# adjerbetian/OpenCL_PathTracer

Hardware: AMD Instinct MI355X
Metric: Msamples/s (paths x bounces) at 1920x1080 (higher is better)
Workload: dtype f32; 1 GPU; BASELINE configs[2]: synthetic random-triangle scene (numpy MT19937 seed 12345): 1000000 triangles (665533 BVH nodes, depth 22), 1920x1080, ray depth 10, JITTERED, 1 light(s); spp_total=256, parallelism=single GPU

## Files before the change

### opencl_pathtracer_amd/csrc/kernel_wavefront.hip

```cpp
#include <hip/hip_runtime.h>

#include "ptmi_device.hpp"
#include "ptmi_shading.hpp"
#include "ptmi_literal_path.hpp"

#include <atomic>
#include <cstdlib>
#include <cstring>

namespace PTMI_DEV_NS {

constexpr int kWfBlock = 256;
constexpr int kWfBlockNarrow = 64;
constexpr int kWfStack = PTMI_BVH_MAX_DEPTH;
#ifndef PTMI_WF_MIN_WAVES
#define PTMI_WF_MIN_WAVES 5
#endif
#ifndef PTMI_WF_MIN_WAVES_GENERAL
#define PTMI_WF_MIN_WAVES_GENERAL 5
#endif
#ifndef PTMI_WF_QUEUES
#define PTMI_WF_QUEUES 8
#endif
constexpr int kQueues = PTMI_WF_QUEUES;
#ifndef PTMI_WF_QUEUE_STRIDE
#define PTMI_WF_QUEUE_STRIDE 64
#endif
constexpr int kQueueStride = PTMI_WF_QUEUE_STRIDE;
static_assert(kQueueStride >= 2, "job_counter[1] is the given-up flag: queue counters must not be adjacent words");
constexpr int kHitRecordWords = 4;
#ifndef PTMI_WF_LEAF_LANES
#define PTMI_WF_LEAF_LANES 19
#endif
#ifndef PTMI_WF_LEAF_RATIO
#define PTMI_WF_LEAF_RATIO 2
#endif
constexpr int kLeafLanes = PTMI_WF_LEAF_LANES, kLeafRatio = PTMI_WF_LEAF_RATIO;
constexpr int kPassWordsPerLane = 4;

struct DWarm {
    const DNode* nodes;
    const DTri* tris;
    const DBigLeaf* big_leaves;
    const uint32_t* tri_ids;
    const DShade* shade;
    const DMat* mats;
    const ptmi_light* lights;
    const ptmi_texture* textures;
    const ptmi_uchar4* texels;
    uint32_t root_ref;
    uint32_t width, height;
    uint32_t max_depth, n_lights, sampler, tris_precomputed;
    uint32_t histograms;
    uint32_t boxes_ordered;
    uint32_t wide_records;
    uint32_t russian_roulette;
    uint32_t source_seed;
    uint32_t wait_debt;
    uint32_t split_paths;
};

constexpr uint32_t kStatDepthBins = 64;
constexpr uint32_t kPoisonMarker = 0x7FC0DEADu;
constexpr uint32_t kGivenUp = 0x80000000u, kGiveUpListFirst = (uint32_t)(kQueues * kQueueStride), kGiveUpListCap = 8u * 1024u - kGiveUpListFirst;
static_assert(kQueues * kQueueStride <= 1024, "the give-up list lies behind the queue counters inside the set's 8 x 1024 dwords");
constexpr uint32_t kSplitWords = C_TRI + 1;
static_assert(PTMI_COUNTER_SPLITS * (int)kSplitWords <= 64, "flushed by one wave");
__device__ __forceinline__ uint32_t counter_split_of(uint32_t slot, uint32_t split_paths)
{
    const uint32_t t1 = split_paths ? split_paths : 0xFFFFFFFFu, t2 = split_paths ? 2u * split_paths : 0xFFFFFFFFu,
                   t3 = split_paths ? 3u * split_paths : 0xFFFFFFFFu;
    return (slot >= t1 ? 1u : 0u) + (slot >= t2 ? 1u : 0u) + (slot >= t3 ? 1u : 0u);
}

__device__ __forceinline__ uint32_t pack_path_statistics(uint32_t depth, uint32_t bbx, uint32_t tri)
{
    static_assert(PTMI_MAX_INTERSECTION_NUMBER <= 8191, "13-bit fields");
    const uint32_t b = bbx < PTMI_MAX_INTERSECTION_NUMBER ? bbx : 8191u, t = tri < PTMI_MAX_INTERSECTION_NUMBER ? tri : 8191u;
    return depth | (b << 6) | (t << 19);
}

__device__ __forceinline__ void decode_leaf(const DWarm& sc, uint32_t ref, uint32_t& tri_i, uint32_t& tri_end)
{
    uint32_t count = (ref >> REF_COUNT_SHIFT) & 7u;
    uint32_t start = ref & REF_INDEX_MASK_LEAF;
    if (count == REF_COUNT_BIG) {
        const DBigLeaf bl = sc.big_leaves[start];
        start = bl.start;
        count = bl.count;
    }
    tri_i = start;
    tri_end = start + count;
}

__device__ __forceinline__ void add_retraced_totals(unsigned long long* totals, uint32_t depth, uint32_t n_seg, uint32_t n_shadow,
                                                    const PathCounters& pc)
{
    atomicAdd(&totals[C_PATHS], 1ull);
    atomicAdd(&totals[C_SEGMENTS], (unsigned long long)n_seg - 1ull);
    atomicAdd(&totals[C_HITS], (unsigned long long)depth);
    atomicAdd(&totals[C_SHADOW], (unsigned long long)n_shadow);
    atomicAdd(&totals[C_BBX], (unsigned long long)pc.bbx);
    atomicAdd(&totals[C_TRI], (unsigned long long)pc.tri);
}

__device__ __forceinline__ void give_path_up(V4& radiance, V4& transfer, uint32_t& reflection, uint32_t& p_bbx, uint32_t& p_tri)
{
    const float m = __uint_as_float(kPoisonMarker);
    radiance = v4(m, m, m, m);
    transfer = v4(1, 1, 1, 1);
    reflection = 0; p_bbx = 0; p_tri = 0;
}

template <bool STATS, bool PRE, bool SS, bool PLAIN = false, bool NANSAFE = false, int BLOCK = 256>
__global__ void __launch_bounds__(BLOCK, PLAIN ? PTMI_WF_MIN_WAVES : PTMI_WF_MIN_WAVES_GENERAL) render_wavefront_kernel(
                                                                    const DScene* __restrict__ scene_in_memory, const DWarm sc_arg, const uint32_t first_iteration,
                                                                    const uint32_t n_iterations, const uint32_t iteration_stride,
                                                                    const uint32_t n_jobs,
                                                                    uint32_t* __restrict__ job_counter,
                                                                    const uint32_t stack_levels,
                                                                    float* __restrict__ stage,
                                                                    uint32_t* __restrict__ stage_stats)
{
    DWarm sc = sc_arg;
    if (PLAIN) { sc.sampler = PTMI_SAMPLER_JITTERED; sc.russian_roulette = 0; sc.n_lights = 1; }
    constexpr bool kOneLight = PLAIN;
    constexpr int kWfBlock = BLOCK;
    constexpr bool kTos = !PLAIN;
    extern __shared__ __attribute__((aligned(16))) uint32_t stack_mem[];
    constexpr uint32_t kBlockCounters = STATS ? (uint32_t)C_COUNT : PTMI_COUNTER_SPLITS * kSplitWords;
    static_assert(kBlockCounters <= 64, "zeroed and flushed by one wave");
    __shared__ unsigned long long block_counters[kBlockCounters];

    const uint32_t tid = threadIdx.x;
    if (tid < kBlockCounters) block_counters[tid] = 0;
    __syncthreads();
    uint32_t* const stack_floor = &stack_mem[kHitRecordWords * kWfBlock + tid];
    *stack_floor = REF_NONE;
    auto cold_scene = [&]() -> const DScene& {
        const DScene* p = scene_in_memory;
        asm volatile("" : "+s"(p));
        return *p;
    };
    uint32_t* const hit_mem = &stack_mem[tid];
    constexpr uint32_t kHitFront = 0x80000000u, kHitFound = 0x40000000u;
    constexpr int kWordS = 1, kWordT = 2, kWordTri = 3;
    const uint32_t tiles_x = (sc.width + 7u) >> 3;
    const bool owns_pixel = sc.sampler != PTMI_SAMPLER_RANDOM;
    const uint32_t n_tiles = (n_jobs / n_iterations) >> 6;
    uint32_t q_cur = blockIdx.x % (uint32_t)kQueues, q_done = 0;

    bool alive = true, need_path = true;
    uint32_t slot = 0;
    int seed = 1;
    V4 transfer = v4(1, 1, 1, 1), radiance = v4(0, 0, 0, 0);
    uint32_t reflection = 0, p_bbx = 0, p_tri = 0;
    bool in_water = false;
    Ray r;
    r.o = v4(0, 0, 0, 0); r.d = v4(0, 0, 0, 0); r.ix = r.iy = r.iz = 0;
    float limit = 0;
    bool shadow = false;
    bool exact_boxes = false;
    bool wave_exact = true;
    uint32_t cur = REF_IDLE, tri_i = 0, tri_end = 0;
    uint32_t dir_signs = 0;
    uint32_t* sp = stack_floor;
    uint32_t tos = REF_NONE;
    auto load_hit_point = [&]() {
        if (shadow) return r.o;
        return mad(r.d, __uint_as_float(hit_mem[0 * kWfBlock]), r.o);
    };
    auto query_found = [&]() {
        return (hit_mem[kWordTri * kWfBlock] & kHitFound) != 0;
    };
    V4 cam_d = v4(0, 0, 0, 0), direct = v4(0, 0, 0, 0);
    uint32_t light_idx = 0;
    uint32_t trips_i = 0, trips_p = 0;
    unsigned long long lanes_i = 0, lanes_p = 0;
    unsigned long long cycles_p = 0;
    const unsigned long long loop_start = STATS ? __builtin_amdgcn_s_memtime() : 0ull;

    auto check = [&](bool holds, int slot) {
        if (STATS && !holds) atomicAdd(&block_counters[slot], 1ull);
    };
    auto finish_path = [&](bool missed) {
        uint32_t split_paths = sc.split_paths;
        asm volatile("" : "+s"(split_paths));
        uint32_t none = STATS ? 0u : counter_split_of(slot, split_paths) * kSplitWords;
        asm volatile("" : "+v"(none));
        unsigned long long* const totals = &block_counters[none];
        atomicAdd(&totals[C_PATHS], 1ull);
        atomicAdd(&totals[C_HITS], (unsigned long long)reflection);
        atomicAdd(&totals[C_SEGMENTS], (unsigned long long)(reflection + (missed ? 1u : 0u)));
        atomicAdd(&totals[C_BBX], (unsigned long long)p_bbx);
        atomicAdd(&totals[C_TRI], (unsigned long long)p_tri);
        check(p_bbx < PTMI_MAX_INTERSECTION_NUMBER && p_tri < PTMI_MAX_INTERSECTION_NUMBER, C_CHK_STATS_RANGE);
        const bool given_up = !owns_pixel && (slot & kGivenUp) != 0u;
        if (sc.histograms && stage_stats == nullptr && !given_up) {
            count_path_in_histograms(cold_scene(), reflection, p_bbx, p_tri);
        }
        if (owns_pixel) {
            reinterpret_cast<float4*>(stage)[slot] = make_float4(radiance.x, radiance.y, radiance.z, radiance.w);
            if (stage_stats != nullptr) stage_stats[slot] = pack_path_statistics(reflection, p_bbx, p_tri);
            if (SS) cold_scene().stage_flag[slot] = 1.f;
        } else if (!given_up) {
            uint32_t gx, gy, it;
            decode_slot(slot, sc.width, sc.width * sc.height, first_iteration, iteration_stride, gx, gy, it);
            int seed0 = lcg_seed(gx, gy, sc.width, sc.height, it, sc.source_seed != 0);
            float sample_x, sample_y;
            draw_sample(sc, gx, gy, it, seed0, sample_x, sample_y);
            const uint32_t off = sample_pixel(sc, sample_x, sample_y);
            add_random_sample(cold_scene(), off, radiance, SS, it);
        }
        need_path = true;
        cur = REF_NONE; tri_i = tri_end = 0;
    };

    auto start_query = [&]() {
        cur = sc.root_ref; sp = stack_floor; tri_i = tri_end = 0;
        if (kTos) tos = REF_NONE;
        if (shadow) atomicAnd(&hit_mem[kWordTri * kWfBlock], ~kHitFound);
        else hit_mem[kWordTri * kWfBlock] = 0;
        exact_boxes = !(sc.boxes_ordered && ray_slabs_are_ordered(r));
        if (cur & REF_LEAF) {
            decode_leaf(sc, cur, tri_i, tri_end);
            cur = REF_NONE;
        }
    };

    unsigned long long* const key_mem = reinterpret_cast<unsigned long long*>(&stack_mem[(kHitRecordWords + 1 + stack_levels) * kWfBlock]);
    uint2* const item_mem = reinterpret_cast<uint2*>(&stack_mem[(kHitRecordWords + 3 + stack_levels) * kWfBlock]) + (tid & ~63u);
    const uint32_t lane = tid & 63u, wave_first = (uint32_t)__builtin_amdgcn_readfirstlane((int)(tid & ~63u));
    uint32_t pass_rounds = 0, pass_items = 0, item_violations = 0;
    const uint32_t n_records = STATS ? cold_scene().n_records : 0u;
    auto leaf_pass = [&](bool waits_at_leaf) {
        auto lanes_below = [&](unsigned long long m) {
            return __builtin_amdgcn_mbcnt_hi((uint32_t)(m >> 32), __builtin_amdgcn_mbcnt_lo((uint32_t)m, 0u));
        };
        const uint32_t left = tri_end - tri_i;
        const uint32_t offered = waits_at_leaf ? (left < 4u ? left : 4u) : 0u;
        const unsigned long long plane0 = __builtin_amdgcn_ballot_w64((offered & 1u) != 0), plane1 = __builtin_amdgcn_ballot_w64((offered & 2u) != 0),
                                 plane2 = __builtin_amdgcn_ballot_w64((offered & 4u) != 0);
        const int n_items = __popcll(plane0) + 2 * __popcll(plane1) + 4 * __popcll(plane2);
        const uint32_t first_item = lanes_below(plane0) + 2u * lanes_below(plane1) + 4u * lanes_below(plane2);
        const uint32_t room = first_item < 64u ? 64u - first_item : 0u;
        const uint32_t cnt = offered < room ? offered : room;
        const uint32_t n_now = n_items < 64 ? (uint32_t)n_items : 64u;
        if (STATS) { pass_rounds++; pass_items += n_now; }
        if (cnt != 0u) {
            key_mem[tid] = shadow ? ~0ull : (((unsigned long long)__float_as_uint(limit) << 32) | 0xFFFFFFFFull);
#pragma unroll
            for (uint32_t j = 0; j < 4u; j++)
                if (j < cnt) item_mem[first_item + j] = make_uint2((tri_i + j) | (shadow ? 0x80000000u : 0u), lane);
        }
        {
            const bool has_item = lane < n_now;
            const uint2 item = has_item ? item_mem[lane] : make_uint2(0u, 0u);
            const uint32_t owner = item.y;
            const int from = (int)(owner << 2);
            auto fetch = [&](float x) { return __int_as_float(__builtin_amdgcn_ds_bpermute(from, __float_as_int(x))); };
            const uint32_t w_tri = item.x & 0x7FFFFFFFu;
            const bool w_shadow = (item.x >> 31) != 0u;
            if (STATS && has_item && (owner >= 64u || w_tri >= n_records)) item_violations++;
            const float4* const rec = reinterpret_cast<const float4*>(&sc.tris[has_item ? w_tri : 0u]);
            constexpr int kE1 = PRE ? 1 : 3, kL0 = PRE ? 2 : 1, kL1 = PRE ? 3 : 2;
            const float4 e0 = rec[0], e1 = rec[kE1];
            asm volatile("" ::: "memory");
            Ray wr;
            wr.o = v4(fetch(r.o.x), fetch(r.o.y), fetch(r.o.z), fetch(r.o.w));
            wr.d = v4(fetch(r.d.x), fetch(r.d.y), fetch(r.d.z), fetch(r.d.w));
            wr.ix = wr.iy = wr.iz = 0;
            const float w_limit = fetch(limit);
            if (has_item) {
                unsigned long long* const owner_key = &key_mem[wave_first + owner];
                tri_test<PRE>(e0, e1, [&](float4& l0, float4& l1) { l0 = rec[kL0]; l1 = rec[kL1]; }, wr, w_limit,
                              [&](const V4&, float ray_t, float s, float t, bool front, float nsd) {
                    const bool nan_hit = NANSAFE && !w_shadow && !(nsd == nsd);
                    const unsigned long long key = w_shadow ? ((unsigned long long)w_tri << 32)
                                                   : nan_hit ? 0ull
                                                   : (((unsigned long long)__float_as_uint(nsd) << 32) | (unsigned long long)(~w_tri));
                    atomicMin(owner_key, key);
                    if (!w_shadow && *owner_key == key) {
                        uint32_t* const rec_out = &stack_mem[wave_first + owner];
                        rec_out[0 * kWfBlock] = __float_as_uint(ray_t);
                        rec_out[kWordS * kWfBlock] = __float_as_uint(s);
                        rec_out[kWordT * kWfBlock] = __float_as_uint(t);
                        rec_out[kWordTri * kWfBlock] = w_tri | (front ? kHitFront : 0u) | kHitFound;
                    }
                });
            }
        }
        if (cnt != 0u) {
            const uint32_t won = (uint32_t)(key_mem[tid] >> 32);
            if (NANSAFE && !shadow && won == 0u) {
                give_path_up(radiance, transfer, reflection, p_bbx, p_tri);
                hit_mem[kWordTri * kWfBlock] = 0;
                cur = REF_NONE; tri_i = tri_end = 0; sp = stack_floor;
                if (kTos) tos = REF_NONE;
                job_counter[1] = 1u;
            } else
            if (!shadow) {
                limit = __uint_as_float(won);
                p_tri += cnt; tri_i += cnt;
            } else if (won != 0xFFFFFFFFu) {
                p_tri += won - tri_i + 1u;
                hit_mem[kWordTri * kWfBlock] |= kHitFound;
                tri_end = tri_i; cur = REF_NONE;
            } else {
                p_tri += cnt; tri_i += cnt;
            }
            if (tri_i >= tri_end && cur != REF_NONE && (cur & REF_LEAF)) {
                decode_leaf(sc, cur, tri_i, tri_end);
                cur = kTos ? tos : *sp;
                uint32_t* const under = sp - kWfBlock;
                sp = under < stack_floor ? stack_floor : under;
                if (kTos) tos = *sp;
            }
        }
    };
    auto node_step = [&]() {
        const float4* const rec = reinterpret_cast<const float4*>(&sc.tris[cur & REF_INDEX_MASK_INNER]);
        const float4 a = rec[0], b = rec[1], c = rec[2], d = rec[3];
        const float lo1[3] = {a.x, a.y, a.z}, hi1[3] = {a.w, b.x, b.y};
        const float lo2[3] = {b.z, b.w, c.x}, hi2[3] = {c.y, c.z, c.w};
        const uint32_t ref1 = __float_as_uint(d.x), ref2 = __float_as_uint(d.y), axis = __float_as_uint(d.z);
        const bool fwd = ((dir_signs >> axis) & 1u) != 0;
        bool h1, h2;
        if (!wave_exact) {
            h1 = box_hit_ordered(lo1, hi1, r, limit);
            h2 = box_hit_ordered(lo2, hi2, r, limit);
        } else {
            h1 = box_hit(lo1, hi1, (ref1 & REF_EMPTY) != 0, r, limit);
            h2 = box_hit(lo2, hi2, (ref2 & REF_EMPTY) != 0, r, limit);
        }
        p_bbx += 2;
        if (kTos) {
            const uint32_t far_ref = fwd ? ref2 : ref1;
            sp[kWfBlock] = far_ref;
            uint32_t* const pushed = sp + kWfBlock;
            const uint32_t child = fwd ? (h1 ? ref1 : ref2) : (h2 ? ref2 : ref1);
            cur = h1 ? child : (h2 ? child : tos);
            tos = h1 ? (h2 ? far_ref : tos) : tos;
            sp = h1 ? (h2 ? pushed : sp) : sp;
            if (!(h1 | h2)) {
                uint32_t* const below = sp - kWfBlock;
                sp = below < stack_floor ? stack_floor : below;
                tos = *sp;
            }
            if (cur != REF_NONE && (cur & REF_LEAF)) {
                decode_leaf(sc, cur, tri_i, tri_end);
                cur = tos;
                uint32_t* const under = sp - kWfBlock;
                sp = under < stack_floor ? stack_floor : under;
                tos = *sp;
            }
            return;
        }
        sp[kWfBlock] = fwd ? ref2 : ref1;
        uint32_t* const pushed = sp + kWfBlock;
        sp = h1 ? (h2 ? pushed : sp) : sp;
        const uint32_t popped = *sp;
        uint32_t* const below = sp - kWfBlock;
        uint32_t* const under = below < stack_floor ? stack_floor : below;
        const uint32_t child = fwd ? (h1 ? ref1 : ref2) : (h2 ? ref2 : ref1);
        cur = h1 ? child : (h2 ? child : popped);
        sp = h1 ? sp : (h2 ? sp : under);
        if (cur != REF_NONE && (cur & REF_LEAF)) {
            decode_leaf(sc, cur, tri_i, tri_end);
            cur = *sp;
            uint32_t* const under = sp - kWfBlock;
            sp = under < stack_floor ? stack_floor : under;
        }
    };

    int wait_debt = 0;
    bool pending, want_inner, want_post;
    int n_t, n_i, n_p;
    bool any_lane;
    unsigned long long dead_lanes = 0ull;
    auto survey = [&]() {
        pending = tri_i < tri_end;
        const bool has_node = cur < REF_DEAD;
        const unsigned long long b_t = __builtin_amdgcn_ballot_w64(pending), b_n = __builtin_amdgcn_ballot_w64(has_node), b_dead = dead_lanes;
        const unsigned long long m_t = b_t, m_i = b_n & ~b_t, m_p = ~(b_t | b_n | b_dead);
        want_inner = !pending & has_node;
        want_post = !pending & !has_node & (cur != REF_DEAD);
        any_lane = (m_t | m_i | m_p) != 0ull;
        n_t = __popcll(m_t); n_i = __popcll(m_i); n_p = __popcll(m_p);
        asm volatile("" : "+s"(n_t), "+s"(n_i));
        wait_debt += n_p;
    };
    const int wait_debt_bound = (int)sc.wait_debt;
    auto path_logic_due = [&]() { return n_p > 0 && wait_debt >= wait_debt_bound; };
    auto nothing_traverses = [&]() { return n_t == 0 && n_i == 0; };
    for (;;) {
        survey();
        if (!any_lane) break;
        auto to_path_logic = [&]() { return path_logic_due() || nothing_traverses(); };
        auto pass_is_due = [&]() { return n_t >= kLeafLanes || (n_t > 0 && 3 * n_t >= kLeafRatio * n_i); };
        while (!to_path_logic()) {
            if (pass_is_due()) {
                leaf_pass(pending);
                survey();
                continue;
            }
            if (STATS) { trips_i++; lanes_i += n_i; }
            if (want_inner) node_step();
            survey();
        }
        wait_debt = 0;
        if (STATS) { trips_p++; lanes_p += n_p; }
        const unsigned long long pass_start = STATS ? __builtin_amdgcn_s_memtime() : 0ull;
        bool new_ray = false;
        V4 new_direction = v4(0, 0, 0, 0);
        if (want_post) {
            need_path = cur == REF_IDLE;
            alive = true;
            bool end_path = false, missed = false;
            bool start_shadow = false, do_scatter = false, lit = false;
            Hit hit;
            hit.point = v4(0, 0, 0, 0); hit.s = hit.t = 0; hit.tri = 0; hit.front = false;
            if (!need_path) {
                hit.point = load_hit_point();
                const bool found = query_found();
                if (!shadow) {
                    if (found) {
                        cam_d = r.d;
                        if (!kOneLight) {
                            direct = v4(0, 0, 0, 0);
                            light_idx = 0;
                        }
                        if (sc.n_lights > 0) start_shadow = true;
                        else do_scatter = true;
                    } else {
                        radiance = mad(sky_color(cold_scene().sky, sc.texels, r.d), transfer, radiance);
                        end_path = missed = true;
                    }
                } else {
                    lit = !found;
                    if (!kOneLight && light_idx + 1u < sc.n_lights) start_shadow = true;
                    else do_scatter = true;
                }
                if (lit || do_scatter) {
                    Surface sf;
                    const uint32_t w6 = hit_mem[kWordTri * kWfBlock];
                    hit.s = __uint_as_float(hit_mem[kWordS * kWfBlock]); hit.t = __uint_as_float(hit_mem[kWordT * kWfBlock]);
                    hit.tri = w6 & REF_INDEX_MASK_LEAF; hit.front = (w6 & kHitFront) != 0;
                    Ray arrival;
                    arrival.o = hit.point; arrival.d = cam_d; arrival.ix = arrival.iy = arrival.iz = 0;
                    load_surface<PLAIN>(sc, arrival, hit, sf);
                    check(dot(cam_d, sf.Ns) < 0 && dot(cam_d, sf.Ng) < 0, C_CHK_NORMALS);
                    V4 gathered = kOneLight ? v4(0, 0, 0, 0) : direct;
                    if (lit) {
                        ptmi_light light = sc.lights[kOneLight ? 0u : light_idx];
                        if (PLAIN) light.type = PTMI_LIGHT_POINT;
                        const float brdf = material_brdf(sf.mat.type, -r.d, sf.Ns, cam_d);
                        gathered = mad(v4(1, 1, 1, 1) * (light_power_toward(light, hit.point, sf.Ns) * brdf), v4(light.color), gathered);
                        if (!kOneLight) direct = gathered;
                        check(gathered.x >= 0 && gathered.y >= 0 && gathered.z >= 0, C_CHK_RADIANCE);
// ... 99 lines not shown
                    uint32_t idx = (uint32_t)n;
                    if (idx > 1000u) idx = 1000u;
                    skip = (double)lcg_random(seed) > (double)fdiv(100 * sigma2_n, cs.x2inv[idx]) + 0.05;
                }
                if (skip) {
                    if (owns_pixel) cold_scene().stage_flag[gy * sc.width + gx] = 0.f;
                    need_path = true;
                } else
                if (sc.max_depth > 0) {
                    limit = INFINITY;
                    new_ray = true;
                } else {
                    finish_path(false);
                }
            }
            if (new_ray) {
                ray_set_direction(r, new_direction);
                dir_signs = (r.d.x > 0 ? 1u : 0u) | (r.d.y > 0 ? 2u : 0u) | (r.d.z > 0 ? 4u : 0u);
                const float o_size = __builtin_fabsf(r.o.x) + __builtin_fabsf(r.o.y) + __builtin_fabsf(r.o.z) + __builtin_fabsf(r.o.w);
                const float d_size = __builtin_fabsf(r.d.x) + __builtin_fabsf(r.d.y) + __builtin_fabsf(r.d.z) + __builtin_fabsf(r.d.w);
                bool bad = !((o_size <= 0x1p+40f) & (d_size <= 4.0f));
                if (!PLAIN && !owns_pixel && __builtin_expect(bad, 0)) {
                    const uint32_t place = atomicAdd(&job_counter[2], 1u);
                    bad = place < kGiveUpListCap;
                    if (bad) {
                        job_counter[kGiveUpListFirst + place] = slot;
                        slot |= kGivenUp;
                    }
                }
                if (__builtin_expect(bad, 0)) {
                    give_path_up(radiance, transfer, reflection, p_bbx, p_tri);
                    shadow = false;
                    job_counter[1] = 1u;
                }
                start_query();
                if (__builtin_expect(bad, 0)) { cur = REF_NONE; tri_i = tri_end = 0; }
            }
            if (need_path) cur = alive ? REF_IDLE : REF_DEAD;
        }
        dead_lanes = __builtin_amdgcn_ballot_w64(cur == REF_DEAD);
        wave_exact = __builtin_amdgcn_ballot_w64(exact_boxes) != 0ull;
        if (STATS) cycles_p += __builtin_amdgcn_s_memtime() - pass_start;
    }

    if (STATS && (tid & 63u) == 0) {
        atomicAdd(&block_counters[C_TRIPS_I], (unsigned long long)trips_i);
        atomicAdd(&block_counters[C_LANES_I], lanes_i);
        atomicAdd(&block_counters[C_TRIPS_T], (unsigned long long)(pass_rounds));
        atomicAdd(&block_counters[C_LANES_T], (unsigned long long)pass_items);
        atomicAdd(&block_counters[C_TRIPS_P], (unsigned long long)trips_p);
        atomicAdd(&block_counters[C_LANES_P], lanes_p);
        atomicAdd(&block_counters[C_CYCLES_P], cycles_p);
        atomicAdd(&block_counters[C_CYCLES_LOOP], __builtin_amdgcn_s_memtime() - loop_start);
    }
    if (STATS && item_violations != 0u) atomicAdd(&block_counters[C_ITEM_VIOLATIONS], (unsigned long long)item_violations);
    __syncthreads();
    if (tid < (STATS ? 1u : (uint32_t)PTMI_COUNTER_SPLITS)) {
        unsigned long long* const totals = &block_counters[tid * kSplitWords];
        totals[C_SHADOW] = totals[C_HITS] * sc.n_lights;
    }
    __syncthreads();
    if (STATS) {
        if (tid < C_COUNT) atomicAdd(&cold_scene().counters[tid], block_counters[tid]);
    } else if (tid < kBlockCounters) {
        const uint32_t k = tid / kSplitWords, c = tid % kSplitWords;
        if (k == 0u || block_counters[tid] != 0ull) atomicAdd(&cold_scene().counters[k * C_COUNT + c], block_counters[tid]);
    }
}

template <bool PRE>
__global__ void __launch_bounds__(kBlock) redo_poisoned_kernel(const DScene sc, const uint32_t first_iteration, const uint32_t n_iterations,
                                                               const uint32_t iteration_stride, float* __restrict__ stage,
                                                               uint32_t* __restrict__ stage_stats, const uint32_t* __restrict__ job_counter)
{
    if (__builtin_nontemporal_load(&job_counter[1]) == 0u) return;
    __shared__ uint32_t stack_mem[kStackDepth * kBlock];
    __shared__ unsigned long long block_counters[PTMI_COUNTER_SPLITS * kSplitWords];
    __shared__ uint32_t queues[kBlock / 64][128];
    const uint32_t tid = threadIdx.x, lane = tid & 63u;
    if (tid < PTMI_COUNTER_SPLITS * kSplitWords) block_counters[tid] = 0;
    __syncthreads();
    const uint32_t n_pixels = sc.width * sc.height, n_slots = n_pixels * n_iterations;
    auto trace_slot = [&](const uint32_t slot) {
        uint32_t gx, gy, it;
        decode_slot(slot, sc.width, n_pixels, first_iteration, iteration_stride, gx, gy, it);
        float sx, sy;
        uint32_t depth = 0, n_seg = 0, n_shadow = 0;
        PathCounters pc;
        const V4 radiance = trace_path<PRE>(sc, gx, gy, it, &stack_mem[tid], sx, sy, depth, n_seg, n_shadow, pc, sc.super_sampling != 0 && it > 5u);
        reinterpret_cast<float4*>(stage)[slot] = make_float4(radiance.x, radiance.y, radiance.z, radiance.w);
        if (stage_stats != nullptr) {
            stage_stats[slot] = pack_path_statistics(depth, pc.bbx, pc.tri);
        } else if (sc.hist_depths) {
            atomicSub(&sc.hist_depths[0], 1u); atomicSub(&sc.hist_bbx[0], 1u); atomicSub(&sc.hist_tri[0], 1u);
            count_path_in_histograms(sc, depth, pc.bbx, pc.tri);
        }
        add_retraced_totals(&block_counters[counter_split_of(slot, sc.split_paths) * kSplitWords], depth, n_seg, n_shadow, pc);
    };
    uint32_t* const queue = queues[tid >> 6];
    uint32_t queued = 0;
    const uint32_t n_waves = gridDim.x * (kBlock / 64), n_chunks = (n_slots + 63u) / 64u;
    for (uint32_t chunk = blockIdx.x * (kBlock / 64) + (tid >> 6); chunk < n_chunks; chunk += n_waves) {
        const uint32_t slot = chunk * 64u + lane;
        bool marked = false;
        if (slot < n_slots) {
            const uint4 v = reinterpret_cast<const uint4*>(stage)[slot];
// ... 109 lines not shown
    const float4 after = make_float4(before.x + r.x, before.y + r.y, before.z + r.z, before.w + r.w);
    const float n_before = image_ray_nb[p];
    const float n_after = n_before + 1.f;
    image_ray_nb[p] = n_after;
    reinterpret_cast<float4*>(image_color)[p] = after;
    float4 v = make_float4(0, 0, 0, 0);
    if (iteration != 0 && n_before != 0.f) {
        v = reinterpret_cast<const float4*>(image_v)[p];
        v.x = mad(r.x - fdiv(before.x, n_before), r.x - fdiv(after.x, n_after), v.x);
        v.y = mad(r.y - fdiv(before.y, n_before), r.y - fdiv(after.y, n_after), v.y);
        v.z = mad(r.z - fdiv(before.z, n_before), r.z - fdiv(after.z, n_after), v.z);
        v.w = mad(r.w - fdiv(before.w, n_before), r.w - fdiv(after.w, n_after), v.w);
    }
    reinterpret_cast<float4*>(image_v)[p] = v;
}

#if PTMI_DEFAULT_ARITHMETIC
__global__ void __launch_bounds__(256) precompute_denominators_kernel(DTri* __restrict__ records, const uint32_t* __restrict__ tri_ids,
                                                                       const uint32_t n_records)
{
    const uint32_t i = blockIdx.x * blockDim.x + threadIdx.x;
    if (i >= n_records || tri_ids[i] == 0xFFFFFFFFu) return;
    DTriPre* const p = reinterpret_cast<DTriPre*>(&records[i]);
    const V4 u = v4(p->u_den[0], p->u_den[1], p->u_den[2], 0.0f), v = v4(p->v_s1w[0], p->v_s1w[1], p->v_s1w[2], 0.0f);
    const float uv = dot(u, v), uu = dot(u, u), vv = dot(v, v);
    p->u_den[3] = frcp(mad(uv, uv, -(uu * vv)));
}
#endif

}

namespace ptmi_internal {

#if PTMI_DEFAULT_ARITHMETIC
int launch_precompute_denominators_da(DTri* records, const uint32_t* tri_ids, uint32_t n_records, void* stream, std::string* err)
{
    if (n_records == 0) return PTMI_OK;
    hipLaunchKernelGGL(PTMI_DEV_NS::precompute_denominators_kernel, dim3((n_records + 255u) / 256u), dim3(256), 0, (hipStream_t)stream,
                       records, tri_ids, n_records);
    return launch_status(hipGetLastError(), "precompute_denominators_kernel", err);
}
#endif

static uint32_t clamp_levels(uint32_t stack_levels)
{
    if (stack_levels < 1) stack_levels = 1;
    if (stack_levels > (uint32_t)PTMI_DEV_NS::kWfStack) stack_levels = PTMI_DEV_NS::kWfStack;
    return stack_levels;
}

static size_t wavefront_lds_bytes(uint32_t stack_levels, int block)
{
    stack_levels = clamp_levels(stack_levels);
    return (size_t)(stack_levels + 1 + PTMI_DEV_NS::kHitRecordWords + PTMI_DEV_NS::kPassWordsPerLane) * block * sizeof(uint32_t);
}

template <class Kernel>
static int resident_blocks_of(Kernel kernel, uint32_t stack_levels, int block)
{
    int device = 0, per_cu = 0, n_cu = 0;
    if (hipGetDevice(&device) != hipSuccess) return 0;
    if (hipDeviceGetAttribute(&n_cu, hipDeviceAttributeMultiprocessorCount, device) != hipSuccess) return 0;
    if (hipOccupancyMaxActiveBlocksPerMultiprocessor(&per_cu, kernel, block, wavefront_lds_bytes(stack_levels, block)) != hipSuccess)
        return 0;
    if (per_cu < 1) per_cu = 1;
    return per_cu * n_cu;
}

static std::atomic<uint32_t> g_last_grid[64];
void PTMI_ARITH(last_wavefront_grid)(int device, uint32_t* lanes, uint32_t* resident)
{
    const uint32_t v = device >= 0 && device < 64 ? g_last_grid[device].load(std::memory_order_relaxed) : 0u;
    *lanes = v >> 20;
    *resident = v & 0xFFFFFu;
}

namespace {

struct WavefrontLaunch {
    int device;
    bool cached_device;
    uint32_t lv, n_jobs;
    hipStream_t st;
    const DScene* scene_in_device_memory;
    PTMI_DEV_NS::DWarm warm;
    uint32_t first_iteration, n_iterations, iteration_stride;
    uint32_t* job_counter;
    float* stage;
    uint32_t* stage_stats;
};
constexpr int kMaxCachedDevices = 64;

static bool five_wide_workgroups_fit(const WavefrontLaunch& w)
{
    static std::atomic<int> wide_fits[kMaxCachedDevices][PTMI_BVH_MAX_DEPTH + 1];
    int fits = w.cached_device ? wide_fits[w.device][w.lv].load(std::memory_order_relaxed) : 0;
    if (fits == 0) {
        int n_cu = 0;
        const int wide = resident_blocks_of(PTMI_DEV_NS::render_wavefront_kernel<false, true, false, true, false>, w.lv, PTMI_DEV_NS::kWfBlock);
        const bool known = hipDeviceGetAttribute(&n_cu, hipDeviceAttributeMultiprocessorCount, w.device) == hipSuccess && n_cu > 0 && wide > 0;
        fits = known && wide < 5 * n_cu ? 2 : 1;
        if (w.cached_device) wide_fits[w.device][w.lv].store(fits, std::memory_order_relaxed);
    }
    return fits == 1;
}

template <bool S, bool P, bool A, bool L, bool N, int B>
static void launch_instance(const WavefrontLaunch& w)
{
    auto kernel = PTMI_DEV_NS::render_wavefront_kernel<S, P, A, L, N, B>;
    static std::atomic<int> resident_cache[kMaxCachedDevices][PTMI_BVH_MAX_DEPTH + 1];
    int resident = w.cached_device ? resident_cache[w.device][w.lv].load(std::memory_order_relaxed) : 0;
    if (resident == 0) {
        resident = resident_blocks_of(kernel, w.lv, B);
        if (w.cached_device) resident_cache[w.device][w.lv].store(resident, std::memory_order_relaxed);
    }
    if (w.cached_device) g_last_grid[w.device].store((uint32_t)B << 20 | (uint32_t)resident, std::memory_order_relaxed);
    uint32_t nb = (w.n_jobs + B - 1) / B;
    if (resident > 0 && nb > (uint32_t)resident) nb = (uint32_t)resident;
    hipLaunchKernelGGL(kernel, dim3(nb), dim3(B), wavefront_lds_bytes(w.lv, B), w.st, w.scene_in_device_memory, w.warm, w.first_iteration,
                       w.n_iterations, w.iteration_stride, w.n_jobs, w.job_counter, w.lv, w.stage, w.stage_stats);
}

using LaunchInstance = void (*)(const WavefrontLaunch&);
static LaunchInstance instance_for(const DScene& sc, bool scheduler_stats, bool plain, bool narrow)
{
    constexpr int kWide = PTMI_DEV_NS::kWfBlock, kNarrow = PTMI_DEV_NS::kWfBlockNarrow;
    const bool pre = sc.tris_precomputed != 0;
    if (sc.super_sampling) return pre ? launch_instance<true, true, true, false, true, kWide> : launch_instance<true, false, true, false, true, kWide>;
    if (scheduler_stats) return pre ? launch_instance<true, true, false, false, true, kWide> : launch_instance<true, false, false, false, true, kWide>;
    if (sc.nan_safe) {
        if (plain) return launch_instance<false, true, false, true, true, kWide>;
        return pre ? launch_instance<false, true, false, false, true, kWide> : launch_instance<false, false, false, false, true, kWide>;
    }
    if (plain)
        return narrow ? launch_instance<false, true, false, true, false, kNarrow> : launch_instance<false, true, false, true, false, kWide>;
    if (pre) return narrow ? launch_instance<false, true, false, false, false, kNarrow> : launch_instance<false, true, false, false, false, kWide>;
    return launch_instance<false, false, false, false, false, kWide>;
}

}

int PTMI_ARITH(launch_render_wavefront)(const DScene& sc, const DScene* scene_in_device_memory, uint32_t first_iteration,
                            uint32_t n_iterations, uint32_t iteration_stride, uint32_t* job_counter, uint32_t stack_levels,
                            bool scheduler_stats, float* stage, uint32_t* stage_stats, void* stream, std::string* err)
{
    if (n_iterations == 0) return PTMI_OK;
    const uint32_t tiles = ((sc.width + 7u) / 8u) * ((sc.height + 7u) / 8u);
    const uint64_t jobs64 = (uint64_t)tiles * 64u * n_iterations;
    if (jobs64 > (sc.sampler == PTMI_SAMPLER_RANDOM ? 0x7FFFFFF0ull : 0xFFFFFFF0ull)) {
        if (err) *err = "too many jobs in one launch";
        return PTMI_ERR_INVALID_ARGUMENT;
    }
    const uint32_t n_jobs = (uint32_t)jobs64;
    hipError_t e = hipMemsetAsync(job_counter, 0, PTMI_DEV_NS::kQueues * PTMI_DEV_NS::kQueueStride * sizeof(uint32_t), (hipStream_t)stream);
    if (e == hipSuccess && sc.sampler == PTMI_SAMPLER_RANDOM) {
        const char* off = std::getenv("PTMI_RANDOM_GIVE_UP");
        if (off && off[0] == '0')
            e = hipMemsetD32Async((hipDeviceptr_t)(job_counter + 2), (int)PTMI_DEV_NS::kGiveUpListCap, 1, (hipStream_t)stream);
    }
    if (e == hipSuccess) {
        WavefrontLaunch w{};
        w.lv = clamp_levels(stack_levels); w.n_jobs = n_jobs; w.st = (hipStream_t)stream;
        w.scene_in_device_memory = scene_in_device_memory;
        w.first_iteration = first_iteration; w.n_iterations = n_iterations; w.iteration_stride = iteration_stride;
        w.job_counter = job_counter; w.stage = stage; w.stage_stats = stage_stats;
        w.cached_device = hipGetDevice(&w.device) == hipSuccess && w.device >= 0 && w.device < kMaxCachedDevices;
        const uint32_t lv = w.lv;
        PTMI_DEV_NS::DWarm& warm = w.warm;
        warm.nodes = sc.nodes; warm.tris = sc.tris; warm.big_leaves = sc.big_leaves; warm.tri_ids = sc.tri_ids; warm.shade = sc.shade;
        warm.mats = sc.mats; warm.lights = sc.lights; warm.textures = sc.textures; warm.texels = sc.texels;
        warm.root_ref = sc.root_ref; warm.width = sc.width; warm.height = sc.height; warm.max_depth = sc.max_depth;
        warm.n_lights = sc.n_lights; warm.sampler = sc.sampler; warm.tris_precomputed = sc.tris_precomputed;
        warm.histograms = sc.hist_depths != nullptr;
        warm.boxes_ordered = sc.boxes_ordered;
        warm.wide_records = sc.wide_records;
        warm.russian_roulette = sc.russian_roulette;
        warm.source_seed = sc.source_seed;
        warm.split_paths = sc.split_paths;
        const bool plain = sc.tris_precomputed && sc.plain_shading && sc.sampler == PTMI_SAMPLER_JITTERED && !sc.russian_roulette &&
                           sc.n_lights == 1 && !sc.super_sampling && !scheduler_stats;
        warm.wait_debt = lv >= 16u ? 768u : (plain ? 320u : 512u);
        const bool narrow = !five_wide_workgroups_fit(w) && std::getenv("PTMI_WIDE_WORKGROUPS") == nullptr;
        instance_for(sc, scheduler_stats, plain, narrow)(w);
        e = hipGetLastError();
        const dim3 redo_block(PTMI_DEV_NS::kBlock);
        if (e == hipSuccess && stage == nullptr && sc.sampler == PTMI_SAMPLER_RANDOM) {
            const auto redo_random = sc.tris_precomputed ? PTMI_DEV_NS::redo_random_kernel<true> : PTMI_DEV_NS::redo_random_kernel<false>;
            hipLaunchKernelGGL(redo_random, dim3(64), redo_block, 0, w.st, sc, first_iteration, n_iterations, iteration_stride, job_counter);
            e = hipGetLastError();
        }
        if (e == hipSuccess && stage != nullptr) {
            const auto redo_poisoned = sc.tris_precomputed ? PTMI_DEV_NS::redo_poisoned_kernel<true> : PTMI_DEV_NS::redo_poisoned_kernel<false>;
            hipLaunchKernelGGL(redo_poisoned, dim3(1024), redo_block, 0, w.st, sc, first_iteration, n_iterations, iteration_stride, stage,
                               stage_stats, job_counter);
            e = hipGetLastError();
        }
    }
    return launch_status(e, "render_wavefront_kernel", err);
}

int PTMI_ARITH(launch_accumulate_staged)(const DScene& sc, uint32_t first_iteration, uint32_t n_iterations, const float* stage,
                             const uint32_t* stage_stats, bool with_histograms, void* stream, std::string* err)
{
    if (n_iterations == 0 || sc.sampler == PTMI_SAMPLER_RANDOM) return PTMI_OK;
    const uint32_t n_pixels = sc.width * sc.height;
    if (sc.super_sampling)
        hipLaunchKernelGGL(PTMI_DEV_NS::accumulate_staged_ss_kernel, dim3((n_pixels + 255u) / 256u), dim3(256), 0,
                           (hipStream_t)stream, sc.image_color, sc.image_ray_nb, sc.image_v, stage, sc.stage_flag, n_pixels, first_iteration);
    else
        hipLaunchKernelGGL(PTMI_DEV_NS::accumulate_staged_kernel, dim3((n_pixels + 255u) / 256u), dim3(256), 0,
                           (hipStream_t)stream, sc.image_color, sc.image_ray_nb, stage, n_pixels, n_iterations);
    const int status = launch_status(hipGetLastError(), "accumulate_staged_kernel", err);
    if (status != PTMI_OK) return status;
    if (with_histograms && stage_stats != nullptr) return PTMI_ARITH(launch_histogram_staged)(sc, n_iterations, stage_stats, stream, err);
    return PTMI_OK;
}

int PTMI_ARITH(launch_histogram_staged)(const DScene& sc, uint32_t n_iterations, const uint32_t* stage_stats, void* stream, std::string* err)
{
    const uint32_t n_slots = sc.width * sc.height * n_iterations;
    uint32_t hb = (n_slots + 1023u) / 1024u;
    if (hb > 512u) hb = 512u;
    hipLaunchKernelGGL(PTMI_DEV_NS::histogram_staged_kernel, dim3(hb), dim3(1024), 0, (hipStream_t)stream, sc.hist_depths,
                       sc.hist_bbx, sc.hist_tri, stage_stats, sc.super_sampling ? sc.stage_flag : nullptr, n_slots);
    return launch_status(hipGetLastError(), "histogram_staged_kernel", err);
}

}
```

### opencl_pathtracer_amd/csrc/ptmi_api.cpp

```cpp
#include <hip/hip_runtime.h>
#include <dlfcn.h>

#include <chrono>
#include <cmath>
#include <limits>
#include <cstdlib>
#include <cstring>
#include <mutex>
#include <string>
#include <utility>
#include <vector>

#include "ptmi.h"
#include "ptmi_internal.h"
#include "scene_layout.h"
#include "scene_refit.h"
#include "launch_schedule.h"

using namespace ptmi_internal;

namespace {
const float kX2inv[1001] = {
#include "x2inv_table.inc"
};
std::mutex g_err_mutex;
std::string g_err;
}

void ptmi_internal::set_global_error(const std::string& msg)
{
    std::lock_guard<std::mutex> lock(g_err_mutex);
    g_err = msg;
}

struct DeviceState {
    int device = 0;
    hipStream_t own_stream = nullptr;
    hipStream_t stream = nullptr;
    hipStream_t copy_stream = nullptr;
    std::vector<void*> allocations;
    float* d_color = nullptr;
    float* d_count = nullptr;
    uint32_t* d_hist = nullptr;
    unsigned long long* d_counters = nullptr;
    uint32_t* d_job_counter = nullptr;
    static constexpr int kStageSets = ptmi_internal::kStageSets;
    float* d_stage[kStageSets] = {};
    size_t stage_cap[kStageSets] = {};
    hipStream_t launch_stream[kStageSets] = {};
    hipEvent_t rendered[kStageSets] = {};
    hipEvent_t stage_free[kStageSets] = {};
    hipEvent_t reuse_after[kStageSets] = {};
    unsigned long long* d_set_counters[kStageSets] = {};
    DScene* d_scene_set[kStageSets] = {};
    LaunchSchedule schedule;
    hipEvent_t previous_call_done = nullptr;
    DScene ds{};
// ... 1026 lines not shown
    if (!ctx->have_scene) return fail(ctx, PTMI_ERR_STATE, "ptmi_read_statistics before ptmi_initialize_memory");
    const uint32_t nd = ctx->cfg.ray_max_depth + 1;
    const size_t words = (size_t)nd + 2 * PTMI_MAX_INTERSECTION_NUMBER;
    std::vector<uint32_t> sum(words, 0u), part(words);
    for (DeviceState& d : ctx->dev) {
        ON_DEVICE(ctx, d);
        HIP_TRY(ctx, hipMemcpyAsync(part.data(), d.d_hist, words * 4, hipMemcpyDeviceToHost, d.stream));
        HIP_TRY(ctx, hipStreamSynchronize(d.stream));
        for (size_t i = 0; i < words; i++) sum[i] += part[i];
    }
    if (depths) std::memcpy(depths, sum.data(), nd * 4);
    if (bbx) std::memcpy(bbx, sum.data() + nd, PTMI_MAX_INTERSECTION_NUMBER * 4);
    if (tri) std::memcpy(tri, sum.data() + nd + PTMI_MAX_INTERSECTION_NUMBER, PTMI_MAX_INTERSECTION_NUMBER * 4);
    return PTMI_OK;
}

static int read_counter_block(ptmi_ctx* ctx, unsigned long long* total)
{
    for (int i = 0; i < C_COUNT; i++) total[i] = 0;
    for (DeviceState& d : ctx->dev) {
        ON_DEVICE(ctx, d);
        unsigned long long h[C_COUNT];
        HIP_TRY(ctx, hipMemcpyAsync(h, d.d_counters, sizeof h, hipMemcpyDeviceToHost, d.stream));
        HIP_TRY(ctx, hipStreamSynchronize(d.stream));
        for (int i = 0; i < C_COUNT; i++) total[i] += h[i];
    }
    return PTMI_OK;
}

int ptmi_get_counters(ptmi_ctx* ctx, ptmi_counters* out)
{
    if (!ctx || !out) return PTMI_ERR_INVALID_ARGUMENT;
    if (!ctx->have_scene) return fail(ctx, PTMI_ERR_STATE, "ptmi_get_counters before ptmi_initialize_memory");
    unsigned long long h[C_COUNT];
    if (int rc = read_counter_block(ctx, h)) return rc;
    out->paths = h[C_PATHS]; out->segments = h[C_SEGMENTS]; out->surface_hits = h[C_HITS];
    out->shadow_rays = h[C_SHADOW]; out->box_tests = h[C_BBX]; out->triangle_tests = h[C_TRI];
    return PTMI_OK;
}

int ptmi_get_scheduler_stats(ptmi_ctx* ctx, ptmi_scheduler_stats* out)
{
    if (!ctx || !out) return PTMI_ERR_INVALID_ARGUMENT;
    if (!ctx->have_scene) return fail(ctx, PTMI_ERR_STATE, "ptmi_get_scheduler_stats before ptmi_initialize_memory");
    unsigned long long h[C_COUNT];
    if (int rc = read_counter_block(ctx, h)) return rc;
    out->trips_node = h[C_TRIPS_I]; out->lanes_node = h[C_LANES_I];
    out->trips_triangle = h[C_TRIPS_T]; out->lanes_triangle = h[C_LANES_T];
    out->trips_path = h[C_TRIPS_P]; out->lanes_path = h[C_LANES_P];
    out->cycles_path = h[C_CYCLES_P]; out->cycles_loop = h[C_CYCLES_LOOP];
    out->leaf_item_violations = h[C_ITEM_VIOLATIONS];
    out->paths_retraced = h[C_RETRACED];
    out->textured_hits = h[C_TEXTURED_HITS];
    uint32_t lanes = 0, resident = 0;
    KERNELS_OF(ctx, last_wavefront_grid)(ctx->dev[0].device, &lanes, &resident);
    out->workgroup_lanes = lanes;
    out->resident_workgroups = resident;
    return PTMI_OK;
}

int ptmi_get_invariant_checks(ptmi_ctx* ctx, ptmi_invariant_checks* out)
{
    if (!ctx || !out) return PTMI_ERR_INVALID_ARGUMENT;
    if (!ctx->have_scene) return fail(ctx, PTMI_ERR_STATE, "ptmi_get_invariant_checks before ptmi_initialize_memory");
    unsigned long long h[C_COUNT];
    if (int rc = read_counter_block(ctx, h)) return rc;
    out->sample_out_of_range = h[C_CHK_SAMPLE]; out->normal_not_facing_ray = h[C_CHK_NORMALS];
    out->negative_direct_radiance = h[C_CHK_RADIANCE]; out->scattered_below_surface = h[C_CHK_HEMISPHERE];
    out->statistics_out_of_range = h[C_CHK_STATS_RANGE];
    out->refraction_undefined_in_reference = h[C_UNDEF_REFRACTION];
    return PTMI_OK;
}

int ptmi_kernel_time(ptmi_ctx* ctx, double* total_ms, uint32_t* n_launches)
{
    if (!ctx) return PTMI_ERR_INVALID_ARGUMENT;
    double ms = 0;
    uint32_t n = 0;
    for (DeviceState& d : ctx->dev) {
        if (int rc = fold_events(ctx, d)) return rc;
        ms += d.kernel_ms;
        n += d.kernel_launches;
        d.kernel_ms = 0;
        d.kernel_launches = 0;
    }
    if (total_ms) *total_ms = ms;
    if (n_launches) *n_launches = n;
    return PTMI_OK;
}

int ptmi_device_accumulators(ptmi_ctx* ctx, void** d_color, void** d_count)
{
    if (!ctx) return PTMI_ERR_INVALID_ARGUMENT;
    if (!ctx->have_scene) return fail(ctx, PTMI_ERR_STATE, "ptmi_device_accumulators before ptmi_initialize_memory");
    if (ctx->n_dev() != 1) return fail(ctx, PTMI_ERR_UNSUPPORTED, "ptmi_device_accumulators on a multi-device context (partial sums)");
    if (d_color) *d_color = ctx->dev[0].ds.image_color;
    if (d_count) *d_count = ctx->dev[0].ds.image_ray_nb;
    return PTMI_OK;
}

int ptmi_device_variance(ptmi_ctx* ctx, void** d_image_v)
{
    if (!ctx || !d_image_v) return PTMI_ERR_INVALID_ARGUMENT;
    if (!ctx->have_scene) return fail(ctx, PTMI_ERR_STATE, "ptmi_device_variance before ptmi_initialize_memory");
    if (ctx->n_dev() != 1) return fail(ctx, PTMI_ERR_UNSUPPORTED, "ptmi_device_variance on a multi-device context (per-device moments)");
    if (!ctx->dev[0].ds.image_v) return fail(ctx, PTMI_ERR_STATE, "no variance accumulator: the context was set up without super_sampling");
// ... 238 lines not shown
```

### opencl_pathtracer_amd/csrc/ptmi_internal.h

```cpp
#pragma once

#include <cstdint>
#include <string>

#include "ptmi.h"
#ifdef __HIPCC__
#include <hip/hip_runtime.h>
#endif

namespace ptmi_internal {

void set_global_error(const std::string& msg);

#ifdef __HIPCC__
inline int launch_status(hipError_t e, const char* kernel, std::string* err)
{
    if (e == hipSuccess) return PTMI_OK;
    if (err) *err = std::string(kernel) + " launch: " + hipGetErrorString(e);
    return PTMI_ERR_HIP;
}
#endif

constexpr uint32_t REF_LEAF = 0x80000000u;
constexpr uint32_t REF_EMPTY = 0x40000000u;
constexpr uint32_t REF_COUNT_SHIFT = 27;
constexpr uint32_t REF_COUNT_BIG = 7;
constexpr uint32_t REF_INDEX_MASK_INNER = 0x3FFFFFFFu;
constexpr uint32_t REF_INDEX_MASK_LEAF = 0x07FFFFFFu;
constexpr uint32_t REF_NONE = 0xFFFFFFFFu;
constexpr uint32_t REF_IDLE = 0xFFFFFFFEu;
constexpr uint32_t REF_DEAD = 0xFFFFFFFDu;

struct DNode {
    float lo1[3], hi1[3];
    float lo2[3], hi2[3];
    uint32_t ref1, ref2;
    uint32_t axis;
    uint32_t pad;
};
static_assert(sizeof(DNode) == 64, "DNode");

struct DTri {
    float s1[4], s2[4], s3[4], n[4];
};
static_assert(sizeof(DTri) == 64, "DTri");

struct DTriPre {
    float n[4], s1d[4], u_den[4], v_s1w[4];
};
static_assert(sizeof(DTriPre) == sizeof(DTri), "DTriPre");

struct DShade {
    float n1[4], n2[4], n3[4];
    float uvp[6];
    float uvn[6];
    uint32_t mat_pos, mat_neg;
    uint32_t pad[2];
};
static_assert(sizeof(DShade) == 112, "DShade");

struct DMat {
    float color[4];
    float opacity;
    int32_t texture_id;
    int32_t type;
    uint32_t is_simple_color;
};
static_assert(sizeof(DMat) == 32, "DMat");

struct DBigLeaf {
    uint32_t start, count;
};

#define PTMI_COUNTER_SPLITS 4

enum CounterSlot {
    C_PATHS = 0, C_SEGMENTS, C_HITS, C_SHADOW, C_BBX, C_TRI,
    C_TRIPS_I, C_LANES_I, C_TRIPS_T, C_LANES_T, C_TRIPS_P, C_LANES_P,
    C_CYCLES_P, C_CYCLES_LOOP,
    C_ITEM_VIOLATIONS,
    C_CHK_SAMPLE,
    C_CHK_NORMALS,
    C_CHK_RADIANCE,
    C_CHK_HEMISPHERE,
    C_CHK_STATS_RANGE,
    C_UNDEF_REFRACTION,
    C_TEXTURED_HITS,
    C_RETRACED,
    C_COUNT
};

struct DScene {
    const DNode* nodes;
    const DTri* tris;
    const DShade* shade;
    const DMat* mats;
    const ptmi_light* lights;
    const ptmi_texture* textures;
    const ptmi_uchar4* texels;
    const DBigLeaf* big_leaves;
    const uint32_t* tri_ids;
    float* image_color;
    float* image_ray_nb;
    uint32_t* hist_depths;
    uint32_t* hist_bbx;
    uint32_t* hist_tri;
    unsigned long long* counters;
    uint32_t split_paths;
    float* image_v;
    const float* x2inv;
    float* stage_flag;
    ptmi_sky sky;
    float cam_pos[4], cam_dir[4], cam_right[4], cam_up[4];
    uint32_t root_ref;
    uint32_t width, height;
    uint32_t max_depth;
    uint32_t n_lights;
    uint32_t sampler;
    uint32_t super_sampling;
    uint32_t tris_precomputed;
    uint32_t plain_shading;
    uint32_t nan_safe;
    uint32_t nan_walk_box_tests, nan_walk_tri_tests, nan_walk_last_tri;
    uint32_t n_records;
    uint32_t wide_records;
    uint32_t boxes_ordered;
    uint32_t russian_roulette;
    uint32_t source_seed;
};

#define PTMI_DECLARE_INTEGRATOR_ENTRY_POINTS(SUFFIX)                                                                             \
                                       \
    int launch_render##SUFFIX(const DScene& sc, uint32_t first_iteration, uint32_t n_iterations, uint32_t iteration_stride,      \
                              void* stream, std::string* err);                                                                  \
                            \
      \
    int launch_render_wavefront##SUFFIX(const DScene& sc, const DScene* scene_in_device_memory, uint32_t first_iteration,        \
                                        uint32_t n_iterations, uint32_t iteration_stride, uint32_t* job_counter,                \
                                        uint32_t stack_levels, bool scheduler_stats, float* stage,                              \
                                        uint32_t* stage_stats, void* stream, std::string* err);                                 \
    void last_wavefront_grid##SUFFIX(int device, uint32_t* lanes_per_workgroup, uint32_t* resident_workgroups);                  \
           \
// ... 22 lines not shown
```

Measured before the change: 970.3 Msamples/s.

## Cache top BVH levels in LDS and shrink leaf-pass scratch layout

Each workgroup copies the top levels of the BVH (up to 31 inner nodes for 256-thread blocks) into LDS at kernel start, rewriting child references to a REF_TOP tag so node_step reads those nodes from LDS instead of global memory. The leaf-pass item buffer is packed into 64-bit words that reuse the key area, cutting pass words per lane from four to two and keeping the total LDS footprint nearly unchanged. Stats counters for per-level top visits are added. The cost is a per-block prologue of global loads and a branch in node traversal, and REF_TOP uses bit 29 of inner refs, which assumes inner node indices stay below that bit.

```diff
diff --git a/opencl_pathtracer_amd/csrc/kernel_wavefront.hip b/opencl_pathtracer_amd/csrc/kernel_wavefront.hip
--- a/opencl_pathtracer_amd/csrc/kernel_wavefront.hip
+++ b/opencl_pathtracer_amd/csrc/kernel_wavefront.hip
@@ -36,7 +36,12 @@
 #define PTMI_WF_LEAF_RATIO 2
 #endif
 constexpr int kLeafLanes = PTMI_WF_LEAF_LANES, kLeafRatio = PTMI_WF_LEAF_RATIO;
-constexpr int kPassWordsPerLane = 4;
+constexpr int kPassWordsPerLane = 2;
+constexpr int kTopWordsPerLane = 2;
+constexpr uint32_t top_levels_of(int block) { return block >= 256 ? 5u : 3u; }
+#ifndef PTMI_WF_TOP_QUAD_MAJOR
+#define PTMI_WF_TOP_QUAD_MAJOR 1
+#endif
 
 struct DWarm {
     const DNode* nodes;
@@ -58,6 +63,7 @@
     uint32_t source_seed;
     uint32_t wait_debt;
     uint32_t split_paths;
+    uint32_t top_levels;
 };
 
 constexpr uint32_t kStatDepthBins = 64;
@@ -134,6 +140,37 @@
 
     const uint32_t tid = threadIdx.x;
     if (tid < kBlockCounters) block_counters[tid] = 0;
+    constexpr uint32_t kTopMax = top_levels_of(BLOCK), kTopSlots = (1u << kTopMax) - 1u;
+    static_assert(kTopSlots * 64u <= (uint32_t)(kTopWordsPerLane * BLOCK) * sizeof(uint32_t) && kTopSlots <= 32u && kTopSlots <= (uint32_t)BLOCK,
+                  "the table fits the two words per lane, a slot number fits five bits, one thread per slot");
+    constexpr uint32_t kTopQuadStride = PTMI_WF_TOP_QUAD_MAJOR ? kTopSlots : 1u, kTopSlotStride = PTMI_WF_TOP_QUAD_MAJOR ? 1u : 4u;
+    float4* const top_mem = reinterpret_cast<float4*>(&stack_mem[(kHitRecordWords + 1 + kPassWordsPerLane + stack_levels) * kWfBlock]);
+    {
+        const uint32_t top_levels = sc.top_levels < kTopMax ? sc.top_levels : kTopMax;
+        auto is_inner = [](uint32_t ref) { return (ref & (REF_LEAF | REF_EMPTY)) == 0u; };
+        if (top_levels != 0u && is_inner(sc.root_ref)) {
+            if (tid < (1u << top_levels) - 1u) {
+                const uint32_t level = 31u - (uint32_t)__builtin_clz(tid + 1u), pos = tid + 1u - (1u << level);
+                uint32_t ref = sc.root_ref;
+                for (uint32_t l = 0; l < level && is_inner(ref); l++) {
+                    const uint32_t* const words = reinterpret_cast<const uint32_t*>(&sc.tris[ref & REF_INDEX_MASK_INNER]);
+                    ref = words[12u + ((pos >> (level - 1u - l)) & 1u)];
+                }
+                if (is_inner(ref)) {
+                    const float4* const rec = reinterpret_cast<const float4*>(&sc.tris[ref & REF_INDEX_MASK_INNER]);
+                    float4 d = rec[3];
+                    if (level + 1u < top_levels) {
+                        if (is_inner(__float_as_uint(d.x))) d.x = __uint_as_float(REF_TOP | (2u * tid + 1u));
+                        if (is_inner(__float_as_uint(d.y))) d.y = __uint_as_float(REF_TOP | (2u * tid + 2u));
+                    }
+                    float4* const slot_mem = top_mem + tid * kTopSlotStride;
+                    slot_mem[0u * kTopQuadStride] = rec[0]; slot_mem[1u * kTopQuadStride] = rec[1];
+                    slot_mem[2u * kTopQuadStride] = rec[2]; slot_mem[3u * kTopQuadStride] = d;
+                }
+            }
+            sc.root_ref = REF_TOP;
+        }
+    }
     __syncthreads();
     uint32_t* const stack_floor = &stack_mem[kHitRecordWords * kWfBlock + tid];
     *stack_floor = REF_NONE;
@@ -176,6 +213,7 @@
     V4 cam_d = v4(0, 0, 0, 0), direct = v4(0, 0, 0, 0);
     uint32_t light_idx = 0;
     uint32_t trips_i = 0, trips_p = 0;
+    uint32_t top_visits[5] = {0, 0, 0, 0, 0};
     unsigned long long lanes_i = 0, lanes_p = 0;
     unsigned long long cycles_p = 0;
     const unsigned long long loop_start = STATS ? __builtin_amdgcn_s_memtime() : 0ull;
@@ -229,7 +267,7 @@
     };
 
     unsigned long long* const key_mem = reinterpret_cast<unsigned long long*>(&stack_mem[(kHitRecordWords + 1 + stack_levels) * kWfBlock]);
-    uint2* const item_mem = reinterpret_cast<uint2*>(&stack_mem[(kHitRecordWords + 3 + stack_levels) * kWfBlock]) + (tid & ~63u);
+    unsigned long long* const item_mem = key_mem + (tid & ~63u);
     const uint32_t lane = tid & 63u, wave_first = (uint32_t)__builtin_amdgcn_readfirstlane((int)(tid & ~63u));
     uint32_t pass_rounds = 0, pass_items = 0, item_violations = 0;
     const uint32_t n_records = STATS ? cold_scene().n_records : 0u;
@@ -248,19 +286,19 @@
         const uint32_t n_now = n_items < 64 ? (uint32_t)n_items : 64u;
         if (STATS) { pass_rounds++; pass_items += n_now; }
         if (cnt != 0u) {
-            key_mem[tid] = shadow ? ~0ull : (((unsigned long long)__float_as_uint(limit) << 32) | 0xFFFFFFFFull);
 #pragma unroll
             for (uint32_t j = 0; j < 4u; j++)
-                if (j < cnt) item_mem[first_item + j] = make_uint2((tri_i + j) | (shadow ? 0x80000000u : 0u), lane);
+                if (j < cnt) item_mem[first_item + j] = ((unsigned long long)lane << 32) | (unsigned long long)((tri_i + j) | (shadow ? 0x80000000u : 0u));
         }
         {
             const bool has_item = lane < n_now;
-            const uint2 item = has_item ? item_mem[lane] : make_uint2(0u, 0u);
-            const uint32_t owner = item.y;
+            const unsigned long long item = has_item ? item_mem[lane] : 0ull;
+            if (cnt != 0u) key_mem[tid] = shadow ? ~0ull : (((unsigned long long)__float_as_uint(limit) << 32) | 0xFFFFFFFFull);
+            const uint32_t owner = (uint32_t)(item >> 32), item_x = (uint32_t)item;
             const int from = (int)(owner << 2);
             auto fetch = [&](float x) { return __int_as_float(__builtin_amdgcn_ds_bpermute(from, __float_as_int(x))); };
-            const uint32_t w_tri = item.x & 0x7FFFFFFFu;
-            const bool w_shadow = (item.x >> 31) != 0u;
+            const uint32_t w_tri = item_x & 0x7FFFFFFFu;
+            const bool w_shadow = (item_x >> 31) != 0u;
             if (STATS && has_item && (owner >= 64u || w_tri >= n_records)) item_violations++;
             const float4* const rec = reinterpret_cast<const float4*>(&sc.tris[has_item ? w_tri : 0u]);
             constexpr int kE1 = PRE ? 1 : 3, kL0 = PRE ? 2 : 1, kL1 = PRE ? 3 : 2;
@@ -319,8 +357,18 @@
         }
     };
     auto node_step = [&]() {
-        const float4* const rec = reinterpret_cast<const float4*>(&sc.tris[cur & REF_INDEX_MASK_INNER]);
-        const float4 a = rec[0], b = rec[1], c = rec[2], d = rec[3];
+        typedef float NativeQuad __attribute__((ext_vector_type(4)));
+        typedef const __attribute__((address_space(3))) NativeQuad LdsQuad;
+        typedef const __attribute__((address_space(1))) NativeQuad MemQuad;
+        NativeQuad a, b, c, d;
+        if (cur & REF_TOP) {
+            LdsQuad* const rec = (LdsQuad*)reinterpret_cast<const NativeQuad*>(top_mem) + (cur & 31u) * kTopSlotStride;
+            a = rec[0u * kTopQuadStride]; b = rec[1u * kTopQuadStride]; c = rec[2u * kTopQuadStride]; d = rec[3u * kTopQuadStride];
+            asm volatile("" ::: "memory");
+        } else {
+            MemQuad* const rec = (MemQuad*)reinterpret_cast<const NativeQuad*>(&sc.tris[cur & REF_INDEX_MASK_INNER]);
+            a = rec[0]; b = rec[1]; c = rec[2]; d = rec[3];
+        }
         const float lo1[3] = {a.x, a.y, a.z}, hi1[3] = {a.w, b.x, b.y};
         const float lo2[3] = {b.z, b.w, c.x}, hi2[3] = {c.y, c.z, c.w};
         const uint32_t ref1 = __float_as_uint(d.x), ref2 = __float_as_uint(d.y), axis = __float_as_uint(d.z);
@@ -404,7 +452,12 @@
                 survey();
                 continue;
             }
-            if (STATS) { trips_i++; lanes_i += n_i; }
+            if (STATS) {
+                trips_i++; lanes_i += n_i;
+                const uint32_t top_slot = want_inner && (cur & REF_TOP) ? (cur & 31u) + 1u : 0u;
+#pragma unroll
+                for (uint32_t l = 0; l < 5u; l++) top_visits[l] += (uint32_t)__popcll(__builtin_amdgcn_ballot_w64((top_slot >> l) == 1u));
+            }
             if (want_inner) node_step();
             survey();
         }
@@ -610,6 +663,7 @@
         atomicAdd(&block_counters[C_LANES_P], lanes_p);
         atomicAdd(&block_counters[C_CYCLES_P], cycles_p);
         atomicAdd(&block_counters[C_CYCLES_LOOP], __builtin_amdgcn_s_memtime() - loop_start);
+        for (int l = 0; l < 5; l++) atomicAdd(&block_counters[C_TOP_VISITS + l], (unsigned long long)top_visits[l]);
     }
     if (STATS && item_violations != 0u) atomicAdd(&block_counters[C_ITEM_VIOLATIONS], (unsigned long long)item_violations);
     __syncthreads();
@@ -825,7 +879,8 @@
 static size_t wavefront_lds_bytes(uint32_t stack_levels, int block)
 {
     stack_levels = clamp_levels(stack_levels);
-    return (size_t)(stack_levels + 1 + PTMI_DEV_NS::kHitRecordWords + PTMI_DEV_NS::kPassWordsPerLane) * block * sizeof(uint32_t);
+    return (size_t)(stack_levels + 1 + PTMI_DEV_NS::kHitRecordWords + PTMI_DEV_NS::kPassWordsPerLane + PTMI_DEV_NS::kTopWordsPerLane) * block *
+           sizeof(uint32_t);
 }
 
 template <class Kernel>
@@ -849,6 +904,12 @@
 }
 
 namespace {
+
+static uint32_t top_levels_allowed()
+{
+    const char* v = std::getenv("PTMI_WF_TOP_LEVELS");
+    return v && v[0] >= '0' && v[0] <= '5' && v[1] == '\0' ? (uint32_t)(v[0] - '0') : 5u;
+}
 
 struct WavefrontLaunch {
     int device;
@@ -951,6 +1012,7 @@
         warm.russian_roulette = sc.russian_roulette;
         warm.source_seed = sc.source_seed;
         warm.split_paths = sc.split_paths;
+        warm.top_levels = top_levels_allowed();
         const bool plain = sc.tris_precomputed && sc.plain_shading && sc.sampler == PTMI_SAMPLER_JITTERED && !sc.russian_roulette &&
                            sc.n_lights == 1 && !sc.super_sampling && !scheduler_stats;
         warm.wait_debt = lv >= 16u ? 768u : (plain ? 320u : 512u);
diff --git a/opencl_pathtracer_amd/csrc/ptmi_api.cpp b/opencl_pathtracer_amd/csrc/ptmi_api.cpp
--- a/opencl_pathtracer_amd/csrc/ptmi_api.cpp
+++ b/opencl_pathtracer_amd/csrc/ptmi_api.cpp
@@ -3,6 +3,7 @@
 
 #include <chrono>
 #include <cmath>
+#include <cstdio>
 #include <limits>
 #include <cstdlib>
 #include <cstring>
@@ -1135,6 +1136,11 @@
     out->leaf_item_violations = h[C_ITEM_VIOLATIONS];
     out->paths_retraced = h[C_RETRACED];
     out->textured_hits = h[C_TEXTURED_HITS];
+    if (std::getenv("PTMI_DUMP_TOP_VISITS") != nullptr) {
+        std::fprintf(stderr, "ptmi top visits: node_steps %llu levels", h[C_BBX] / 2ull);
+        for (int l = 0; l < 5; l++) std::fprintf(stderr, " %llu", h[C_TOP_VISITS + l]);
+        std::fprintf(stderr, "\n");
+    }
     uint32_t lanes = 0, resident = 0;
     KERNELS_OF(ctx, last_wavefront_grid)(ctx->dev[0].device, &lanes, &resident);
     out->workgroup_lanes = lanes;
diff --git a/opencl_pathtracer_amd/csrc/ptmi_internal.h b/opencl_pathtracer_amd/csrc/ptmi_internal.h
--- a/opencl_pathtracer_amd/csrc/ptmi_internal.h
+++ b/opencl_pathtracer_amd/csrc/ptmi_internal.h
@@ -27,6 +27,7 @@
 constexpr uint32_t REF_COUNT_BIG = 7;
 constexpr uint32_t REF_INDEX_MASK_INNER = 0x3FFFFFFFu;
 constexpr uint32_t REF_INDEX_MASK_LEAF = 0x07FFFFFFu;
+constexpr uint32_t REF_TOP = 0x20000000u;
 constexpr uint32_t REF_NONE = 0xFFFFFFFFu;
 constexpr uint32_t REF_IDLE = 0xFFFFFFFEu;
 constexpr uint32_t REF_DEAD = 0xFFFFFFFDu;
@@ -87,7 +88,8 @@
     C_UNDEF_REFRACTION,
     C_TEXTURED_HITS,
     C_RETRACED,
-    C_COUNT
+    C_TOP_VISITS,
+    C_COUNT = C_TOP_VISITS + 5
 };
 
 struct DScene {
```

Result: slower. 955.4 Msamples/s (-1.5%).
